# cv-stuttgart/PCFA

Measured on AMD Instinct MI355X. Metric: attack_steps_per_sec, higher is better.
Workload: dtype f32; 1 GPU; RAFT, 1 synthetic 436x1024 pair per GPU (padded 440x1024), disjoint delta, change_of_variables, delta_bound=0.005, zero target, L-BFGS max_iter=10; weights=random:1234, parallelism=pairs sharded 1/GPU, closure_launch=hipGraph replay

## Files before the change

include/pcfa_hip.h:

```cpp
#ifndef PCFA_HIP_H
#define PCFA_HIP_H

#include <stddef.h>
#include <stdint.h>

#ifdef __cplusplus
extern "C" {
#endif

#define PCFA_OK 0
#define PCFA_ERR_INVALID_ARG (-1)
#define PCFA_ERR_UNSUPPORTED (-2)
#define PCFA_ERR_WORKSPACE (-3)

#if defined(__GNUC__)
#define PCFA_API __attribute__((visibility("default")))
#else
#define PCFA_API
#endif

#define PCFA_MAX_LEVELS 8
#define PCFA_ABI_VERSION 2

#define PCFA_LOSS_AEE 0
// ... 82 lines not shown
                        int N, int d, float scale, void* stream);
PCFA_API int pcfa_attn_stream_delta(const float* g, const float* out, float* delta, long long rows, int d,
                           int accumulate, void* stream);
PCFA_API int pcfa_attn_stream_dqk(const float* q, const float* k, const float* lse, const float* G, const float* V,
                         const float* delta, float* dq, float* dk, int BH, int N, int d, int n, float scale,
                         void* stream);

PCFA_API long long pcfa_lookup_convc1_packed_floats(int Cout);
PCFA_API int pcfa_lookup_convc1_pack_weights(const float* weight, float* packed, int Cout, int Cin, void* stream);
PCFA_API int pcfa_lookup_convc1_fwd(const float* pyr, const float* coords, const float* packed, const float* bias,
                           float* out, int B, int H, int W, int num_levels, int radius, int Cout, int relu,
                           void* stream);
PCFA_API int pcfa_lookup_convc1_bwd(float* dpyr, const float* coords, const float* packed, const float* out,
                           const float* grad_out, int B, int H, int W, int num_levels, int radius, int Cout,
                           int relu, void* stream);

PCFA_API int pcfa_spatial_corr_out_size(int iH, int iW, int kH, int kW, int padH, int padW, int dilH,
                               int dilW, int dH, int dW, int* oH, int* oW);
PCFA_API int pcfa_spatial_corr_fwd(const float* in1, const float* in2, float* out, int B, int C, int iH,
                          int iW, int kH, int kW, int patchH, int patchW, int padH, int padW,
                          int dilH, int dilW, int dil_patchH, int dil_patchW, int dH, int dW,
                          void* stream);
PCFA_API int pcfa_spatial_corr_bwd(const float* in1, const float* in2, const float* grad_out,
                          float* grad_in1, float* grad_in2, int B, int C, int iH, int iW, int kH,
                          int kW, int patchH, int patchW, int padH, int padW, int dilH, int dilW,
                          int dil_patchH, int dil_patchW, int dH, int dW, void* stream);

PCFA_API int pcfa_cost_volume9_fwd(const float* in1, const float* in2, float* out, int B, int C, int iH, int iW,
                          float scale, float slope, void* stream);
PCFA_API int pcfa_cost_volume9_bwd(const float* in1, const float* in2, const float* fwd_out, const float* grad_out,
// ... 285 lines not shown
```

pcfa_amd/_hip.py:

```python
import ctypes
import os
from ctypes import c_char_p, c_double, c_float, c_int, c_longlong, c_size_t, c_uint, c_void_p, POINTER

ABI_VERSION = 2
LIB_PATH = os.environ.get("PCFA_HIP_LIB") or os.path.join(os.path.dirname(os.path.abspath(__file__)), "lib",
                                                          "libpcfa_hip.so")

PCFA_LOSS = {"aee": 0, "mse": 1, "cosim": 2}


class HipLibraryError(RuntimeError):
    pass


_P = c_void_p
_S4 = POINTER(c_longlong)

SIGNATURES = {
    "pcfa_abi_version": (c_int, []),
    "pcfa_timing_arm": (c_int, [_P, _P, c_int]),
    "pcfa_null_launch": (c_int, [_P]),
    "pcfa_poison_lds": (c_int, [c_uint, _P]),
    "pcfa_peek_lds": (c_int, [_P, c_int, _P]),
    "pcfa_calib_mfma_f32": (c_longlong, [_P, c_int, c_int, _P]),
# ... 27 lines not shown
    "pcfa_gemm_bf16x3_workspace_bytes": (c_size_t, [c_int, c_int, c_int, c_int]),
    "pcfa_gemm_bf16x3": (c_int, [_P, _P, _P, c_int, c_int, c_int, c_longlong, c_longlong, c_longlong, c_int, c_int,
                                 c_int, c_longlong, c_longlong, c_longlong, c_float, c_int, _P, c_size_t, _P]),
    "pcfa_corr_pyramid_fwd_bf16x3": (c_int, [_P, _P, _P, c_int, c_int, c_int, c_int, c_int, _P]),
    "pcfa_softmax_rows_fwd": (c_int, [_P, _P, c_longlong, c_int, _P]),
    "pcfa_softmax_rows_bwd": (c_int, [_P, _P, _P, c_longlong, c_int, _P]),
    "pcfa_attn_stream_lse": (c_int, [_P, _P, _P, c_int, c_int, c_int, c_float, _P]),
    "pcfa_attn_stream_fwd": (c_int, [_P, _P, _P, _P, _P, c_int, c_int, c_int, c_float, _P]),
    "pcfa_attn_stream_dv": (c_int, [_P, _P, _P, _P, _P, c_int, c_int, c_int, c_float, _P]),
    "pcfa_attn_stream_delta": (c_int, [_P, _P, _P, c_longlong, c_int, c_int, _P]),
    "pcfa_attn_stream_dqk": (c_int, [_P, _P, _P, _P, _P, _P, _P, _P, c_int, c_int, c_int, c_int, c_float, _P]),
    "pcfa_lookup_convc1_packed_floats": (c_longlong, [c_int]),
    "pcfa_lookup_convc1_pack_weights": (c_int, [_P, _P, c_int, c_int, _P]),
    "pcfa_lookup_convc1_fwd": (c_int, [_P, _P, _P, _P, _P, c_int, c_int, c_int, c_int, c_int, c_int, c_int, _P]),
    "pcfa_lookup_convc1_bwd": (c_int, [_P, _P, _P, _P, _P, c_int, c_int, c_int, c_int, c_int, c_int, c_int, _P]),
    "pcfa_spatial_corr_out_size": (c_int, [c_int] * 10 + [POINTER(c_int), POINTER(c_int)]),
    "pcfa_spatial_corr_fwd": (c_int, [_P, _P, _P] + [c_int] * 16 + [_P]),
    "pcfa_spatial_corr_bwd": (c_int, [_P, _P, _P, _P, _P] + [c_int] * 16 + [_P]),
    "pcfa_cost_volume9_fwd": (c_int, [_P, _P, _P, c_int, c_int, c_int, c_int, c_float, c_float, _P]),
    "pcfa_cost_volume9_bwd": (c_int, [_P, _P, _P, _P, _P, _P, c_int, c_int, c_int, c_int, c_float, c_float, _P]),
    "pcfa_flownet_corr_out_size": (c_int, [c_int] * 7 + [POINTER(c_int)] * 3),
    "pcfa_flownet_corr_fwd": (c_int, [_P, _P, _P] + [c_int] * 9 + [_P]),
    "pcfa_flownet_corr_bwd": (c_int, [_P, _P, _P, _P, _P] + [c_int] * 9 + [_P]),
    "pcfa_resample2d_fwd": (c_int, [_P, _P, _P] + [c_int] * 8 + [_P]),
    "pcfa_resample2d_bwd": (c_int, [_P, _P, _P, _P, _P] + [c_int] * 8 + [_P]),
    "pcfa_channelnorm_fwd": (c_int, [_P, _P, c_int, c_int, c_longlong, c_int, _P]),
    "pcfa_channelnorm_bwd": (c_int, [_P, _P, _P, _P, c_int, c_int, c_longlong, c_int, _P]),
    "pcfa_box_transform_fwd": (c_int, [_P, _P, _P, c_int, c_longlong, c_int, c_double, c_float, _P]),
    "pcfa_box_transform_bwd": (c_int, [_P, _P, _P, _P, _P, c_int, c_longlong, c_int, c_double, c_float, _P]),
    "pcfa_pm1_pair_fwd": (c_int, [_P, _P, _P, _P, c_int, c_longlong, _P]),
# ... 169 lines not shown
```

pcfa_amd/config.py:

```python
import dataclasses
import os


def _env_bool(name, default):
    v = os.environ.get(name)
    return default if v is None else v not in ("0", "", "false", "False")


@dataclasses.dataclass(frozen=True)
class Config:
    fused_lookup: bool = True
    overlap_encoders: bool = False
    conv_s2: bool = True
    conv_s2_bwd: bool = True
    fused_downsample: bool = True
    defer_relu: bool = True
    pyramid_bwd_windows: bool = True
    gma_gemm: str = "lib"
    gma_attention: str = "materialised"
    conv1x1: str = "lib"
    corr: str = "all_pairs"
    ondemand_lookup: str = "per_query"
    motion_bwd: str = "batched"
    mfma: str = "f32"
    dilated_as_subgrids: tuple = (2, 4, 8, 16)
    deconv_fewout: bool = True
    defer_leaky: bool = True
    dense_block_fused_masks: bool = True
    warp_bwd_deterministic: bool = True
    pwc_fold_glue: bool = True
    spynet_ops: str = "lib"
    flownet2_ops: str = "lib"
    reuse_pair_graphs: bool = True
    max_cached_shapes: int = 4

    @classmethod
    def from_env(cls):
        return cls(fused_lookup=_env_bool("PCFA_FUSED_LOOKUP", True),
# ... 11 lines not shown
                   max_cached_shapes=int(os.environ.get("PCFA_MAX_CACHED_SHAPES", "4")))

    def __post_init__(self):
        if self.gma_gemm not in ("lib", "hip"):
            raise ValueError("Config.gma_gemm must be 'lib' or 'hip', got %r" % (self.gma_gemm,))
        if self.gma_attention not in ("materialised", "streamed"):
            raise ValueError("Config.gma_attention must be 'materialised' or 'streamed', got %r" % (self.gma_attention,))
        if self.conv1x1 not in ("lib", "hip"):
            raise ValueError("Config.conv1x1 must be 'lib' or 'hip', got %r" % (self.conv1x1,))
        if self.corr not in ("all_pairs", "on_demand"):
            raise ValueError("Config.corr must be 'all_pairs' or 'on_demand', got %r" % (self.corr,))
        if self.ondemand_lookup not in ("per_query", "tiled"):
            raise ValueError("Config.ondemand_lookup must be 'per_query' or 'tiled', got %r" % (self.ondemand_lookup,))
        if self.motion_bwd not in ("batched", "per_iteration"):
            raise ValueError("Config.motion_bwd must be 'batched' or 'per_iteration', got %r" % (self.motion_bwd,))
        if self.mfma not in ("f32", "bf16x3"):
            raise ValueError("Config.mfma must be 'f32' or 'bf16x3', got %r" % (self.mfma,))
        if self.spynet_ops not in ("lib", "hip"):
            raise ValueError("Config.spynet_ops must be 'lib' or 'hip', got %r" % (self.spynet_ops,))
        if self.flownet2_ops not in ("lib", "hip"):
            raise ValueError("Config.flownet2_ops must be 'lib' or 'hip', got %r" % (self.flownet2_ops,))
        if self.max_cached_shapes < 1:
            raise ValueError("Config.max_cached_shapes must be >= 1")


DEFAULT = Config.from_env()


def attach(model, config=None):
    config = DEFAULT if config is None else config
# ... 10 lines not shown
```

pcfa_amd/csrc/corr_lookup_conv.hip:

```cpp
#include <cstdlib>
#include "common.hpp"

namespace {

typedef float f32x4 __attribute__((ext_vector_type(4)));
typedef float f32x16 __attribute__((ext_vector_type(16)));

constexpr int R = 4, N1 = 9, WIN = 10, TXN = 4, PIECES = WIN * TXN;
constexpr int RS = 20, WS = WIN * RS + 4, NRD = 3;
constexpr int QT = 32;
constexpr int NT = 256;
constexpr int NTF = NT + 64;
constexpr int NPC = QT * PIECES / NT;
constexpr int L = 4, TAPS = N1 * N1;
constexpr int KL = 88, KG = KL / 8;
constexpr int KP = L * KL;
constexpr int WIN_FLOATS = QT * WS + 4;
#ifndef PCFA_LC_WD
#define PCFA_LC_WD 8
#endif
#ifndef PCFA_LC_WDB
#define PCFA_LC_WDB 6
#endif
#ifndef PCFA_LC_EARLY
// ... 384 lines not shown
#pragma unroll
    for (int r = 0; r < 16; ++r) {
      const int n = (mt0 + m) * 32 + (r & 3) + 8 * (r >> 2) + 4 * lh;
      float y = acc[m][r];
      if (relu) y = fmaxf(y, 0.f);
      if (qlive) ob[(size_t)n * Q] = y;
    }
  if (dbg & 8) {
    PCFA_LC_STAMP();
    __syncthreads();
    if (tid == 0)
      for (int k = 0; k < 8; ++k) out[(size_t)b_img * COUT * Q + (size_t)k * Q + q0] = (float)(ts[k] - ts[0]);
  }
}

__global__ __launch_bounds__(NT) void corr_lookup_convc1_bwd_kernel(
    float* __restrict__ dpyr, const float* __restrict__ coords, const float* __restrict__ wt,
    const float* __restrict__ y, const float* __restrict__ grad_out, int Q, PyrLayout P, int relu) {
  constexpr int COUT = 256, MT = KP / 32;
  constexpr int MTW = 3;
  __shared__ __attribute__((aligned(16))) float s_a[COUT * QT > WIN_FLOATS ? COUT * QT : WIN_FLOATS];
  __shared__ __attribute__((aligned(16))) float s_dt[KP][QT];
  float (*s_g)[QT] = reinterpret_cast<float (*)[QT]>(s_a);
  float* s_win = s_a;

  const int tid = threadIdx.x, lane = tid & 63, wv = __builtin_amdgcn_readfirstlane(tid >> 6);
  const int j = tid & 31, l31 = lane & 31, lh = lane >> 5;
  const int b_img = blockIdx.z, q0 = blockIdx.x * QT;
  unsigned long long ts[12] = {};
  int nts = 0;
  constexpr int dbg = PCFA_LC_DBG_BUILD;
  PCFA_LC_STAMP();
  const int kq = tid >> 3, sub = tid & 7;
  const bool klive = q0 + kq < Q;
  const float* cb = coords + (size_t)b_img * 2 * Q;
  const int qj = min(q0 + j, Q - 1), qk = min(q0 + kq, Q - 1);
  const float cx = cb[qj], cy = cb[Q + qj], kx = cb[qk], ky = cb[Q + qk];
  float* slab0 = scalar_ptr(dpyr + ((size_t)b_img * Q + q0) * P.slab);

  const int qq = (tid & 7) * 4, n0 = tid >> 3;
  const size_t gbase = (size_t)b_img * COUT * Q + q0 + qq;
  const bool full = __builtin_amdgcn_readfirstlane((Q & 3) == 0 && q0 + QT <= Q);
  constexpr int NBLK = COUT / 32, AHEAD = PCFA_LC_AHEAD;
  f32x4 gg[NBLK], yy[NBLK];
  const float* ysrc = relu ? y : grad_out;
  const size_t glast = (size_t)gridDim.z * COUT * Q - 4;
  auto tile_load = [&](int i) {
    const size_t o = min(gbase + (size_t)(n0 + 32 * i) * Q, glast);
    gg[i] = *reinterpret_cast<const f32x4*>(grad_out + o);
    yy[i] = *reinterpret_cast<const f32x4*>(ysrc + o);
  };
  auto tile_store = [&](int i) {
    f32x4 t;
    t.x = (yy[i].x > 0.f || !relu) ? gg[i].x : 0.f; t.y = (yy[i].y > 0.f || !relu) ? gg[i].y : 0.f;
    t.z = (yy[i].z > 0.f || !relu) ? gg[i].z : 0.f; t.w = (yy[i].w > 0.f || !relu) ? gg[i].w : 0.f;
    *reinterpret_cast<f32x4*>(&s_g[n0 + 32 * i][qq]) = t;
  };
#pragma unroll
  for (int i = 0; i < AHEAD; ++i) tile_load(i);
  __builtin_amdgcn_sched_barrier(0);
// ... 25 lines not shown
    const int hl = Ph[l], wl = Pw[l], tw = Ptw[l], ox = org[l].ox;
    const int y = org[l].y0 + rr, gtx = (org[l].x0 >> 2) + tx;
    const bool need = (unsigned)y < (unsigned)hl && (unsigned)gtx < (unsigned)tw && 4 * tx < ox + WIN;
    const int c0 = 4 * tx - ox, gx0 = 4 * gtx;
    int mask = need ? 16 : 0;
#pragma unroll
    for (int e = 0; e < 4; ++e)
      if ((unsigned)(c0 + e) < (unsigned)WIN && gx0 + e < wl) mask |= 1 << e;
    pmask[l][i] = mask;
    pgoff[l][i] = need ? org[l].wB + (((((unsigned)y >> 2) * (unsigned)tw + (unsigned)gtx) << 4) + (((unsigned)y & 3u) << 2)) * 4u
                       : (unsigned)Pzero * 4u;
    plds[l][i] = (unsigned)(kq * WS + rr * RS + 4 + 4 * tx - ox) * 4u;
  };
  __builtin_amdgcn_sched_barrier(0);
  PCFA_LC_STAMP();
  if (!full) {
#pragma unroll 1
    for (int i = 0; i < NBLK; ++i) {
      const size_t o = gbase + (size_t)(n0 + 32 * i) * Q;
#pragma unroll
      for (int e = 0; e < 4; ++e) {
        const bool ok = q0 + qq + e < Q;
        const float gv = ok ? grad_out[o + e] : 0.f;
        const float yv = (ok && relu) ? y[o + e] : 1.f;
        s_g[n0 + 32 * i][qq + e] = yv > 0.f ? gv : 0.f;
      }
    }
  }

  {
    f32x16 acc[MTW];
#pragma unroll
    for (int m = 0; m < MTW; ++m)
#pragma unroll
      for (int r = 0; r < 16; ++r) acc[m][r] = 0.f;
    const f32x4* wq = reinterpret_cast<const f32x4*>(wt) + lane;
    const int nmt = wv + 8 < MT ? 3 : 2;
    constexpr int WD = PCFA_LC_WDB, NGB = COUT / 8;
    f32x4 wring[WD][MTW];
    size_t wrow[MTW];
#pragma unroll
    for (int m = 0; m < MTW; ++m) wrow[m] = (size_t)min(wv + 4 * m, MT - 1) * NGB;
#pragma unroll
    for (int d = 0; d < WD; ++d)
#pragma unroll
      for (int m = 0; m < MTW; ++m) wring[d][m] = wq[(wrow[m] + d) * 64];
    float bv[4] = {0.f, 0.f, 0.f, 0.f};
#pragma unroll
    for (int g = 0; g < NGB; ++g) {
      if (g % 4 == 0) {
        if (full) tile_store(g / 4);
        __syncthreads();
        if (g == 0) PCFA_LC_STAMP();
#pragma unroll
        for (int e = 0; e < 4; ++e) bv[e] = s_g[8 * g + 2 * e + lh][l31];
      }
      float bvn[4] = {0.f, 0.f, 0.f, 0.f};
      f32x4 wcur[MTW];
#pragma unroll
      for (int m = 0; m < MTW; ++m) wcur[m] = wring[g % WD][m];
#pragma unroll
      for (int e = 0; e < 4; ++e)
#pragma unroll
        for (int m = 0; m < MTW; ++m) {
          const int step = e * MTW + m;
          const float av = e == 0 ? wcur[m].x : e == 1 ? wcur[m].y : e == 2 ? wcur[m].z : wcur[m].w;
          acc[m] = __builtin_amdgcn_mfma_f32_32x32x2f32(av, bv[e], acc[m], 0, 0, 0);
          if (step == 0 && (g + 1) % 4 != 0) {
#pragma unroll
            for (int ee = 0; ee < 4; ++ee) bvn[ee] = s_g[8 * (g + 1) + 2 * ee + lh][l31];
          }
          if (step == 4 && g % 4 == 0 && g / 4 + AHEAD < NBLK) tile_load(g / 4 + AHEAD);
          if (step == 1 && g + WD < NGB) {
#pragma unroll
            for (int mm = 0; mm < MTW; ++mm) wring[g % WD][mm] = wq[(wrow[mm] + g + WD) * 64];
          }
          if (step == 2 && g < L * NPC && g % NPC == 0) level_setup(g / NPC);
          if (step == 3 && g < L * NPC) piece_setup(g / NPC, g % NPC);
          if (step == 5 && g < L * NPC) v[g / NPC][g % NPC] = load_piece(slab0, pgoff[g / NPC][g % NPC]);
          __builtin_amdgcn_sched_barrier(0);
        }
#pragma unroll
      for (int e = 0; e < 4; ++e) bv[e] = bvn[e];
    }
#pragma unroll
    for (int m = 0; m < MTW; ++m) {
      if (m < nmt) {
#pragma unroll
        for (int r = 0; r < 16; ++r)
          s_dt[(wv + 4 * m) * 32 + (r & 3) + 8 * (r >> 2) + 4 * lh][l31] = acc[m][r];
      }
    }
  }
  __syncthreads();
  PCFA_LC_STAMP();

#pragma unroll
  for (int l = 0; l < L; ++l) {
    const Origin oj = make_origin(cx, cy, l);
    const float fx = oj.fx, fy = oj.fy;
    const float w00 = (1.f - fx) * (1.f - fy), w01 = fx * (1.f - fy), w10 = (1.f - fx) * fy, w11 = fx * fy;
#pragma unroll
    for (int pass = 0; pass < 2; ++pass) {
      const int row = pass == 0 ? (tid >> 5) : 8;
      if (pass == 1 && tid >= 32) break;
      float gc[N1], gp[N1];
#pragma unroll
      for (int a = 0; a < N1; ++a) {
        gc[a] = s_dt[l * KL + a * N1 + row][j];
        gp[a] = row > 0 ? s_dt[l * KL + a * N1 + row - 1][j] : 0.f;
      }
      float4* dst0 = reinterpret_cast<float4*>(&s_win[j * WS + row * RS + 4]);
      float d[NRD * 4];
#pragma unroll
      for (int c = 0; c < NRD * 4; ++c) {
        float s = 0.f;
        if (c < N1) s = gc[c] * w00;
        if (c >= 1 && c <= N1) s = fmaf(gc[c - 1], w01, s);
        if (c < N1) s = fmaf(gp[c], w10, s);
        if (c >= 1 && c <= N1) s = fmaf(gp[c - 1], w11, s);
        d[c] = s;
      }
#pragma unroll
      for (int i = 0; i < NRD; ++i) dst0[i] = make_float4(d[4 * i], d[4 * i + 1], d[4 * i + 2], d[4 * i + 3]);
      if (row == N1 - 1) {
        float4* dst1 = reinterpret_cast<float4*>(&s_win[j * WS + (WIN - 1) * RS + 4]);
#pragma unroll
        for (int c = 0; c < NRD * 4; ++c) {
          float s = 0.f;
          if (c < N1) s = gc[c] * w10;
          if (c >= 1 && c <= N1) s = fmaf(gc[c - 1], w11, s);
          d[c] = s;
        }
#pragma unroll
        for (int i = 0; i < NRD; ++i) dst1[i] = make_float4(d[4 * i], d[4 * i + 1], d[4 * i + 2], d[4 * i + 3]);
      }
    }
    __syncthreads();
    const char* lds_bytes = reinterpret_cast<const char*>(s_win);
#pragma unroll
    for (int i = 0; i < NPC; ++i) {
      const float* src = reinterpret_cast<const float*>(lds_bytes + plds[l][i]);
      const float e0 = src[0], e1 = src[1], e2 = src[2], e3 = src[3];
      const int m = pmask[l][i];
      f32x4 t = v[l][i];
      t.x += (m & 1) ? e0 : 0.f;
      t.y += (m & 2) ? e1 : 0.f;
      t.z += (m & 4) ? e2 : 0.f;
      t.w += (m & 8) ? e3 : 0.f;
      if (m & 16) store_piece(slab0, pgoff[l][i], t);
    }
    __syncthreads();
    PCFA_LC_STAMP();
  }
  if (dbg & 8) {
    if (tid == 0)
      for (int k = 0; k < 8; ++k) slab0[k] = (float)(ts[k] - ts[0]);
  }
}

bool check_levels(const PyrLayout& P) {
  for (int l = 0; l < P.L; ++l)
    if (P.h[l] < 1 || P.w[l] < 1 || P.h[l] > 32000 || P.w[l] > 32000) return false;
  return true;
}

}

extern "C" long long pcfa_lookup_convc1_packed_floats(int Cout) {
  if (Cout != 256) return -1;
  return 2LL * Cout * KP;
}

// ... 23 lines not shown

extern "C" int pcfa_lookup_convc1_bwd(float* dpyr, const float* coords, const float* packed, const float* out,
                                      const float* grad_out, int B, int H, int W, int num_levels, int radius,
                                      int Cout, int relu, void* stream) {
  PyrLayout P;
  if (!dpyr || !coords || !packed || !out || !grad_out || B < 1 || !pcfa_make_layout(P, H, W, num_levels) ||
      !check_levels(P))
    return PCFA_ERR_INVALID_ARG;
  if (num_levels != L || radius != R || Cout != 256) return PCFA_ERR_UNSUPPORTED;
  const int Q = H * W;
  pcfa_launch(corr_lookup_convc1_bwd_kernel, dim3(pcfa_cdiv(Q, QT), 1, B), dim3(NT), 0, (hipStream_t)stream, dpyr,
              coords, packed + (size_t)Cout * KP, out, grad_out, Q, P, relu);
  PCFA_LAUNCH_CHECK();
  return PCFA_OK;
}
```

pcfa_amd/nets/raft.py:

```python

import torch
import torch.nn as nn
import torch.nn.functional as F

from .. import ops
from ..config import cfg


def _norm(kind, planes):
    if kind == 'batch':
        return nn.BatchNorm2d(planes)
    if kind == 'instance':
        return nn.InstanceNorm2d(planes)
    if kind == 'group':
        return nn.GroupNorm(num_groups=planes // 8, num_channels=planes)
    if kind == 'none':
        return nn.Sequential()
    raise ValueError("unknown norm_fn %r" % kind)


def _fold_batchnorm(conv, bn, cache, tag):
    tensors = (conv.weight, conv.bias, bn.weight, bn.bias, bn.running_mean, bn.running_var)
    key = tuple((t.data_ptr(), t._version) for t in tensors if t is not None) + (conv.weight.device,)
    hit = cache.get(tag)
# ... 359 lines not shown
class BasicUpdateBlock(nn.Module):
    def __init__(self, corr_levels=4, corr_radius=4, hidden_dim=128):
        super().__init__()
        self.encoder = BasicMotionEncoder(corr_levels, corr_radius)
        self.gru = SepConvGRU(hidden_dim=hidden_dim, input_dim=128 + hidden_dim)
        self.flow_head = FlowHead(hidden_dim, hidden_dim=256)
        self.mask = _mask_head()
        self._mask_cache = {}

    def motion_steps(self, corr_fn, flow, iters, gru_ctx):
        c, enc = cfg(self), self.encoder
        make = getattr(ops.get(), "motion_steps", None)
        if (make is None or c.motion_bwd != "batched" or not c.defer_relu or not c.fused_lookup or c.corr == "on_demand"
                or gru_ctx is None or not flow.is_cuda or not enc.can_defer_relu(flow)):
            return None
        return make(corr_fn, iters, *((m.weight, m.bias) for m in (enc.convc1, enc.convc2, enc.convf1, enc.convf2, enc.conv)))

    def forward(self, net, inp, corr, flow, want_mask=True, gru_ctx=None, motion=None):
        if motion is not None:
            steps, itr = motion
            net = self.gru.step(net, gru_ctx, steps.step(itr, corr.coords, flow), self.encoder.RELU_CHANNELS,
                                d_rest_dst=steps.d_rest_dst(itr))
        else:
            defer = cfg(self).defer_relu and gru_ctx is not None and self.encoder.can_defer_relu(flow)
            motion_features = self.encoder(flow, corr, defer_relu=defer)
            if gru_ctx is not None:
                net = self.gru.step(net, gru_ctx, motion_features, self.encoder.RELU_CHANNELS if defer else 0)
            else:
                net = self.gru(net, torch.cat([inp, motion_features], dim=1))
        delta_flow = self.flow_head(net)
        mask = mask_logits(self.mask, net, self._mask_cache) if want_mask else None
# ... 91 lines not shown
```

pcfa_amd/ops/corr.py:

```python
import ctypes
import os

import torch

from .. import _hip
from . import core
from .conv import FEWIN_SHAPES, _conv3x3_cat_fill, _conv3x3_packed, _conv3x3_run, conv_fewin
from .core import _call, _dev, _note_work, _pair, _ptr, _ptr_off, _stream, cached_pack


class _CorrState:
    __slots__ = ("B", "D", "H", "W", "L", "r", "slab", "pyr", "f2ext", "dpyr", "token_grad", "coords_bwd", "bwd_windows", "mfma")


class _CorrBuild(torch.autograd.Function):

    @staticmethod
    def forward(ctx, fmap1, fmap2, state):
        lib = _hip.load()
        B, D, H, W = fmap1.shape
        f1 = fmap1.contiguous()
        f2 = fmap2.contiguous()
        slab = state.slab
        state.f2ext = torch.empty((B, D, slab), device=f1.device, dtype=torch.float32)
# ... 122 lines not shown
        if ctx.needs_input_grad[3] or ctx.needs_input_grad[4]:
            raise RuntimeError("lookup_conv is the frozen-weight path: no weight / bias gradient")
        st = ctx.state
        c, out = ctx.saved_tensors
        if st.dpyr is None:
            st.dpyr = torch.zeros_like(st.pyr)
            st.coords_bwd = []
        st.coords_bwd.append(c)
        g = grad_out.contiguous()
        _call("pcfa_lookup_convc1_bwd", _ptr(st.dpyr), _ptr(c), _ptr(ctx.packed), _ptr(out), _ptr(g), st.B, st.H, st.W,
              st.L, st.r, ctx.cout, ctx.relu)
        return _token_grad(st, g.device), None, None, None, None, None


class _MotionState:
    __slots__ = ("iters", "H", "W", "corr", "w", "cor1", "cf", "rest", "d_rest", "coords", "arrived", "token_grad", "packs")


def _slab_image(slab, i):
    n = slab[0].numel()
    return torch.empty(0, device=slab.device, dtype=slab.dtype).set_(
        slab.untyped_storage(), slab.storage_offset() + i * n, (1,) + tuple(slab.shape[1:]))


class _MotionFlush(torch.autograd.Function):

    @staticmethod
    def forward(ctx, token, ms):
        ctx.ms = ms
        return token.view_as(token)

# ... 15 lines not shown
        direct = lambda b, k, n_: (lib.pcfa_conv3x3_algo(b, k, n_, H, W) == 23
                                   and lib.pcfa_conv3x3_workspace_bytes(b, k, n_, H, W) == 0)
        batched = (len(live) == n and all(direct(b, k, n_) for b in (1, n)
                                          for k, n_ in ((n_c, k_c), (n_c, n_c2), (n_c2, k_c2))))
        d_cor1 = torch.empty((n, k_c2, H, W), device=dev, dtype=torch.float32)
        if batched:
            d_cf = torch.empty((n, n_c2, H, W), device=dev, dtype=torch.float32)
            _call("pcfa_conv3x3_run_strided", _ptr(ms.d_rest), wr * plane, _ptr(bwd_c), None, _ptr(ms.cf), k_c * plane, None, 0,
                  _ptr(d_cf), n_c2 * plane, n, n_c, n_c2, H, W, 0, 0., 0, None, ctypes.c_size_t(0))
            _call("pcfa_conv3x3_run_strided", _ptr(d_cf), n_c2 * plane, _ptr(bwd_c2), None, _ptr(ms.cor1), k_c2 * plane, None, 0,
                  _ptr(d_cor1), k_c2 * plane, n, n_c2, k_c2, H, W, 0, 0., 0, None, ctypes.c_size_t(0))
        if st.dpyr is None:
            st.dpyr = torch.zeros_like(st.pyr)
            st.coords_bwd = []
        packed = _convc1_packed(ms.w["convc1"][0])
        for i in reversed(live):
            if not batched:
                d_cf = torch.empty((1, k_c, H, W), device=dev, dtype=torch.float32)
                _conv3x3_run(dev, _ptr_off(ms.d_rest, i * wr * plane), bwd_c, None, _ptr_off(ms.cf, i * k_c * plane), None,
                             _ptr(d_cf), 1, n_c, k_c, H, W)
                _conv3x3_run(dev, _ptr(d_cf), bwd_c2, None, _ptr_off(ms.cor1, i * k_c2 * plane), None,
                             _ptr_off(d_cor1, i * k_c2 * plane), 1, n_c2, k_c2, H, W)
            st.coords_bwd.append(ms.coords[i])
            _call("pcfa_lookup_convc1_bwd", _ptr(st.dpyr), _ptr(ms.coords[i]), _ptr(packed), _ptr_off(ms.cor1, i * k_c2 * plane),
                  _ptr_off(d_cor1, i * k_c2 * plane), st.B, st.H, st.W, st.L, st.r, k_c2, 1)
        return grad_token, None


class _MotionStep(torch.autograd.Function):

    @staticmethod
    def forward(ctx, token, coords, flow, ms, i):
        st = ms.corr
        c = coords.contiguous()
        (wc1, bc1), (wc2, bc2), (wf1, bf1), (wf2, bf2), (wc, bc) = (ms.w[k] for k in ("convc1", "convc2", "convf1", "convf2", "conv"))
        cor1, cf, rest = _slab_image(ms.cor1, i), _slab_image(ms.cf, i), _slab_image(ms.rest, i)
        _call("pcfa_lookup_convc1_fwd", _ptr(st.pyr), _ptr(c), _ptr(_convc1_packed(wc1)), _ptr(bc1), _ptr(cor1), st.B, st.H,
              st.W, st.L, st.r, wc1.shape[0], 1)
        flo1 = conv_fewin(flow, wf1, bf1, True)
        _conv3x3_cat_fill([cor1, flo1.contiguous()], [wc2, wf2], [bc2, bf2], (), cf)
# ... 24 lines not shown
        self._ms, self._token = ms, token

    def step(self, i, coords, flow):
        _dev(coords, flow)
        if coords.requires_grad and torch.is_grad_enabled():
            raise RuntimeError("motion_steps: coords.requires_grad is not supported (detach the coordinates, as "
                               "models/raft/raft.py:122-123 does)")
        if flow.requires_grad and torch.is_grad_enabled():
            raise RuntimeError("motion_steps: the flow must be detached (models/raft/raft.py:122-123)")
        return _MotionStep.apply(self._token, coords, flow, self._ms, i)

    def d_rest_dst(self, i):
        return _slab_image(self._ms.d_rest, i)


def motion_steps(corr_block, iters, convc1, convc2, convf1, convf2, conv):
    if not isinstance(corr_block, CorrBlock) or iters < 1:
        return None
    st = corr_block._state
    (wc1, bc1), (wc2, bc2), (wf1, bf1), (wf2, bf2), (wc, bc) = convc1, convc2, convf1, convf2, conv
    if (st.B != 1 or st.L != 4 or st.r != 4 or bc1 is None or tuple(wc1.shape) != (256, 324, 1, 1)
            or not corr_block._token.requires_grad
            or any(t is None or t.requires_grad for t in (wc1, bc1, wc2, bc2, wf1, bf1, wf2, bf2, wc, bc))
            or any(tuple(w.shape[2:]) != (3, 3) for w in (wc2, wf2, wc))
            or (wf1.shape[1], wf1.shape[2]) not in FEWIN_SHAPES or wf1.shape[2] != wf1.shape[3]
            or wc2.shape[1] != wc1.shape[0] or wf2.shape[1] != wf1.shape[0] or wc.shape[1] != wc2.shape[0] + wf2.shape[0]):
        return None
    dev = st.pyr.device
    ms = _MotionState()
    ms.iters, ms.H, ms.W, ms.corr = iters, st.H, st.W, st
    ms.w = {"convc1": convc1, "convc2": convc2, "convf1": convf1, "convf2": convf2, "conv": conv}
    new = lambda c: torch.empty((iters, c, st.H, st.W), device=dev, dtype=torch.float32)
    ms.cor1, ms.cf = new(wc1.shape[0]), new(wc.shape[1])
    ms.rest, ms.d_rest = new(wc.shape[0] + 2), new(wc.shape[0] + 2)
    ms.coords, ms.arrived, ms.token_grad = [None] * iters, [False] * iters, None
    ms.packs = ((_conv3x3_packed(wc)[1], wc.shape[1], wc.shape[0]), (_conv3x3_packed(wc2)[1], wc2.shape[1], wc2.shape[0]))
    return MotionSteps(ms, _MotionFlush.apply(corr_block._token, ms))


class CorrBlock:

    def __init__(self, fmap1, fmap2, num_levels=4, radius=4, bwd_windows=True, mfma="f32"):
        _dev(fmap1, fmap2)
        if mfma not in ("f32", "bf16x3"):
            raise ValueError("CorrBlock: mfma must be 'f32' or 'bf16x3', got %r" % (mfma,))
        if fmap1.shape != fmap2.shape or fmap1.dim() != 4:
            raise ValueError("CorrBlock expects two [B,D,H,W] feature maps of equal shape")
        lib = _hip.load()
        self.num_levels = num_levels
        self.radius = radius
# ... 136 lines not shown
```

Before: 7.891 attack_steps/s.

## Fuse per-iteration lookup-convc1 backward launches into one multi-step kernel

Adds a multi-step variant of the lookup+convc1 backward kernel that loops over all RAFT iterations inside one launch. Each block keeps its dpyr slab tile resident and prefetches the next step's coords, gradient tiles and weight ring while it finishes the current step's scatter. This replaces roughly one launch per GRU iteration with a single launch and overlaps the step prologues. In exchange the kernel carries a larger by-value argument struct, extra fences, and more register pressure. It only applies when B==1 and there are at most 32 steps.

```diff
diff --git a/include/pcfa_hip.h b/include/pcfa_hip.h
--- a/include/pcfa_hip.h
+++ b/include/pcfa_hip.h
@@ -120,6 +120,9 @@
 PCFA_API int pcfa_lookup_convc1_bwd(float* dpyr, const float* coords, const float* packed, const float* out,
                            const float* grad_out, int B, int H, int W, int num_levels, int radius, int Cout,
                            int relu, void* stream);
+PCFA_API int pcfa_lookup_convc1_bwd_steps(float* dpyr, const float* const* coords, const long long* offsets,
+                           int nsteps, const float* packed, const float* out, const float* grad_out, int B, int H,
+                           int W, int num_levels, int radius, int Cout, int relu, void* stream);
 
 PCFA_API int pcfa_spatial_corr_out_size(int iH, int iW, int kH, int kW, int padH, int padW, int dilH,
                                int dilW, int dH, int dW, int* oH, int* oW);
diff --git a/pcfa_amd/_hip.py b/pcfa_amd/_hip.py
--- a/pcfa_amd/_hip.py
+++ b/pcfa_amd/_hip.py
@@ -65,6 +65,8 @@
     "pcfa_lookup_convc1_pack_weights": (c_int, [_P, _P, c_int, c_int, _P]),
     "pcfa_lookup_convc1_fwd": (c_int, [_P, _P, _P, _P, _P, c_int, c_int, c_int, c_int, c_int, c_int, c_int, _P]),
     "pcfa_lookup_convc1_bwd": (c_int, [_P, _P, _P, _P, _P, c_int, c_int, c_int, c_int, c_int, c_int, c_int, _P]),
+    "pcfa_lookup_convc1_bwd_steps": (c_int, [_P, POINTER(c_void_p), POINTER(c_longlong), c_int, _P, _P, _P, c_int, c_int,
+                                             c_int, c_int, c_int, c_int, c_int, _P]),
     "pcfa_spatial_corr_out_size": (c_int, [c_int] * 10 + [POINTER(c_int), POINTER(c_int)]),
     "pcfa_spatial_corr_fwd": (c_int, [_P, _P, _P] + [c_int] * 16 + [_P]),
     "pcfa_spatial_corr_bwd": (c_int, [_P, _P, _P, _P, _P] + [c_int] * 16 + [_P]),
diff --git a/pcfa_amd/config.py b/pcfa_amd/config.py
--- a/pcfa_amd/config.py
+++ b/pcfa_amd/config.py
@@ -22,6 +22,7 @@
     corr: str = "all_pairs"
     ondemand_lookup: str = "per_query"
     motion_bwd: str = "batched"
+    lookup_bwd: str = "steps"
     mfma: str = "f32"
     dilated_as_subgrids: tuple = (2, 4, 8, 16)
     deconv_fewout: bool = True
@@ -63,6 +64,8 @@
             raise ValueError("Config.ondemand_lookup must be 'per_query' or 'tiled', got %r" % (self.ondemand_lookup,))
         if self.motion_bwd not in ("batched", "per_iteration"):
             raise ValueError("Config.motion_bwd must be 'batched' or 'per_iteration', got %r" % (self.motion_bwd,))
+        if self.lookup_bwd not in ("steps", "per_iteration"):
+            raise ValueError("Config.lookup_bwd must be 'steps' or 'per_iteration', got %r" % (self.lookup_bwd,))
         if self.mfma not in ("f32", "bf16x3"):
             raise ValueError("Config.mfma must be 'f32' or 'bf16x3', got %r" % (self.mfma,))
         if self.spynet_ops not in ("lib", "hip"):
diff --git a/pcfa_amd/csrc/corr_lookup_conv.hip b/pcfa_amd/csrc/corr_lookup_conv.hip
--- a/pcfa_amd/csrc/corr_lookup_conv.hip
+++ b/pcfa_amd/csrc/corr_lookup_conv.hip
@@ -422,9 +422,29 @@
   }
 }
 
-__global__ __launch_bounds__(NT) void corr_lookup_convc1_bwd_kernel(
-    float* __restrict__ dpyr, const float* __restrict__ coords, const float* __restrict__ wt,
-    const float* __restrict__ y, const float* __restrict__ grad_out, int Q, PyrLayout P, int relu) {
+constexpr int MAX_STEPS = 32;
+struct OneStep {
+  const float *coords_, *y_, *grad_;
+  __device__ __forceinline__ int count() const { return 1; }
+  __device__ __forceinline__ const float* coords(int) const { return coords_; }
+  __device__ __forceinline__ const float* y(int) const { return y_; }
+  __device__ __forceinline__ const float* grad(int) const { return grad_; }
+};
+struct LookupSteps {
+  const float* coords_[MAX_STEPS];
+  long long off[MAX_STEPS];
+  const float *y_, *grad_;
+  int n;
+  __device__ __forceinline__ int count() const { return n; }
+  __device__ __forceinline__ const float* coords(int s) const { return coords_[s]; }
+  __device__ __forceinline__ const float* y(int s) const { return y_ + off[s]; }
+  __device__ __forceinline__ const float* grad(int s) const { return grad_ + off[s]; }
+};
+
+template <bool STEPS, typename Src>
+__device__ __forceinline__ void lookup_convc1_bwd_body(float* __restrict__ dpyr, const Src& src,
+                                                       const float* __restrict__ wt, int Q, const PyrLayout& P,
+                                                       int relu) {
   constexpr int COUT = 256, MT = KP / 32;
   constexpr int MTW = 3;
   __shared__ __attribute__((aligned(16))) float s_a[COUT * QT > WIN_FLOATS ? COUT * QT : WIN_FLOATS];
@@ -437,13 +457,21 @@
   const int b_img = blockIdx.z, q0 = blockIdx.x * QT;
   unsigned long long ts[12] = {};
   int nts = 0;
-  constexpr int dbg = PCFA_LC_DBG_BUILD;
+  constexpr int dbg = STEPS ? (PCFA_LC_DBG_BUILD & ~8) : PCFA_LC_DBG_BUILD;
   PCFA_LC_STAMP();
   const int kq = tid >> 3, sub = tid & 7;
   const bool klive = q0 + kq < Q;
-  const float* cb = coords + (size_t)b_img * 2 * Q;
   const int qj = min(q0 + j, Q - 1), qk = min(q0 + kq, Q - 1);
-  const float cx = cb[qj], cy = cb[Q + qj], kx = cb[qk], ky = cb[Q + qk];
+  const int nsteps = STEPS ? __builtin_amdgcn_readfirstlane(src.count()) : 1;
+  float cx, cy, kx, ky;
+  float ncx = 0.f, ncy = 0.f, nkx = 0.f, nky = 0.f;
+  auto coords_load = [&](int s, float& ax, float& ay, float& bx, float& by) {
+    const float* cb = src.coords(s) + (size_t)b_img * 2 * Q;
+    ax = cb[qj]; ay = cb[Q + qj]; bx = cb[qk]; by = cb[Q + qk];
+  };
+  coords_load(0, cx, cy, kx, ky);
+  const float* grad_out = src.grad(0);
+  const float* y = src.y(0);
   float* slab0 = scalar_ptr(dpyr + ((size_t)b_img * Q + q0) * P.slab);
 
   const int qq = (tid & 7) * 4, n0 = tid >> 3;
@@ -452,6 +480,11 @@
   constexpr int NBLK = COUT / 32, AHEAD = PCFA_LC_AHEAD;
   f32x4 gg[NBLK], yy[NBLK];
   const float* ysrc = relu ? y : grad_out;
+  auto step_sources = [&](int s) {
+    grad_out = src.grad(s);
+    y = src.y(s);
+    ysrc = relu ? y : grad_out;
+  };
   const size_t glast = (size_t)gridDim.z * COUT * Q - 4;
   auto tile_load = [&](int i) {
     const size_t o = min(gbase + (size_t)(n0 + 32 * i) * Q, glast);
@@ -507,149 +540,191 @@
   };
   __builtin_amdgcn_sched_barrier(0);
   PCFA_LC_STAMP();
-  if (!full) {
+  constexpr int WD = PCFA_LC_WDB, NGB = COUT / 8;
+  const f32x4* wq = reinterpret_cast<const f32x4*>(wt) + lane;
+  const int nmt = wv + 8 < MT ? 3 : 2;
+  f32x4 wring[WD][MTW];
+  size_t wrow[MTW];
+#pragma unroll
+  for (int m = 0; m < MTW; ++m) wrow[m] = (size_t)min(wv + 4 * m, MT - 1) * NGB;
+  auto ring_fill = [&]() {
+    if (STEPS) asm volatile("" : "+v"(wq));
+#pragma unroll
+    for (int d = 0; d < WD; ++d)
+#pragma unroll
+      for (int m = 0; m < MTW; ++m) wring[d][m] = wq[(wrow[m] + d) * 64];
+  };
+
 #pragma unroll 1
-    for (int i = 0; i < NBLK; ++i) {
-      const size_t o = gbase + (size_t)(n0 + 32 * i) * Q;
-#pragma unroll
-      for (int e = 0; e < 4; ++e) {
-        const bool ok = q0 + qq + e < Q;
-        const float gv = ok ? grad_out[o + e] : 0.f;
-        const float yv = (ok && relu) ? y[o + e] : 1.f;
-        s_g[n0 + 32 * i][qq + e] = yv > 0.f ? gv : 0.f;
+  for (int s = 0; s < nsteps; ++s) {
+    if (!full) {
+#pragma unroll 1
+      for (int i = 0; i < NBLK; ++i) {
+        const size_t o = gbase + (size_t)(n0 + 32 * i) * Q;
+#pragma unroll
+        for (int e = 0; e < 4; ++e) {
+          const bool ok = q0 + qq + e < Q;
+          const float gv = ok ? grad_out[o + e] : 0.f;
+          const float yv = (ok && relu) ? y[o + e] : 1.f;
+          s_g[n0 + 32 * i][qq + e] = yv > 0.f ? gv : 0.f;
+        }
       }
     }
-  }
-
-  {
-    f32x16 acc[MTW];
-#pragma unroll
-    for (int m = 0; m < MTW; ++m)
-#pragma unroll
-      for (int r = 0; r < 16; ++r) acc[m][r] = 0.f;
-    const f32x4* wq = reinterpret_cast<const f32x4*>(wt) + lane;
-    const int nmt = wv + 8 < MT ? 3 : 2;
-    constexpr int WD = PCFA_LC_WDB, NGB = COUT / 8;
-    f32x4 wring[WD][MTW];
-    size_t wrow[MTW];
-#pragma unroll
-    for (int m = 0; m < MTW; ++m) wrow[m] = (size_t)min(wv + 4 * m, MT - 1) * NGB;
-#pragma unroll
-    for (int d = 0; d < WD; ++d)
-#pragma unroll
-      for (int m = 0; m < MTW; ++m) wring[d][m] = wq[(wrow[m] + d) * 64];
-    float bv[4] = {0.f, 0.f, 0.f, 0.f};
-#pragma unroll
-    for (int g = 0; g < NGB; ++g) {
-      if (g % 4 == 0) {
-        if (full) tile_store(g / 4);
-        __syncthreads();
-        if (g == 0) PCFA_LC_STAMP();
-#pragma unroll
-        for (int e = 0; e < 4; ++e) bv[e] = s_g[8 * g + 2 * e + lh][l31];
+
+    {
+      f32x16 acc[MTW];
+#pragma unroll
+      for (int m = 0; m < MTW; ++m)
+#pragma unroll
+        for (int r = 0; r < 16; ++r) acc[m][r] = 0.f;
+      if (!STEPS || s == 0) ring_fill();
+      float bv[4] = {0.f, 0.f, 0.f, 0.f};
+#pragma unroll
+      for (int g = 0; g < NGB; ++g) {
+        if (g % 4 == 0) {
+          if (full) tile_store(g / 4);
+          __syncthreads();
+          if (g == 0) PCFA_LC_STAMP();
+#pragma unroll
+          for (int e = 0; e < 4; ++e) bv[e] = s_g[8 * g + 2 * e + lh][l31];
+        }
+        float bvn[4] = {0.f, 0.f, 0.f, 0.f};
+        f32x4 wcur[MTW];
+#pragma unroll
+        for (int m = 0; m < MTW; ++m) wcur[m] = wring[g % WD][m];
+#pragma unroll
+        for (int e = 0; e < 4; ++e)
+#pragma unroll
+          for (int m = 0; m < MTW; ++m) {
+            const int step = e * MTW + m;
+            const float av = e == 0 ? wcur[m].x : e == 1 ? wcur[m].y : e == 2 ? wcur[m].z : wcur[m].w;
+            acc[m] = __builtin_amdgcn_mfma_f32_32x32x2f32(av, bv[e], acc[m], 0, 0, 0);
+            if (step == 0 && (g + 1) % 4 != 0) {
+#pragma unroll
+              for (int ee = 0; ee < 4; ++ee) bvn[ee] = s_g[8 * (g + 1) + 2 * ee + lh][l31];
+            }
+            if (step == 4 && g % 4 == 0 && g / 4 + AHEAD < NBLK) tile_load(g / 4 + AHEAD);
+            if (step == 1 && g + WD < NGB) {
+#pragma unroll
+              for (int mm = 0; mm < MTW; ++mm) wring[g % WD][mm] = wq[(wrow[mm] + g + WD) * 64];
+            }
+            if (step == 2 && g < L * NPC && g % NPC == 0) level_setup(g / NPC);
+            if (step == 3 && g < L * NPC) piece_setup(g / NPC, g % NPC);
+            if (step == 5 && g < L * NPC) v[g / NPC][g % NPC] = load_piece(slab0, pgoff[g / NPC][g % NPC]);
+            __builtin_amdgcn_sched_barrier(0);
+          }
+#pragma unroll
+        for (int e = 0; e < 4; ++e) bv[e] = bvn[e];
       }
-      float bvn[4] = {0.f, 0.f, 0.f, 0.f};
-      f32x4 wcur[MTW];
-#pragma unroll
-      for (int m = 0; m < MTW; ++m) wcur[m] = wring[g % WD][m];
-#pragma unroll
-      for (int e = 0; e < 4; ++e)
-#pragma unroll
-        for (int m = 0; m < MTW; ++m) {
-          const int step = e * MTW + m;
-          const float av = e == 0 ? wcur[m].x : e == 1 ? wcur[m].y : e == 2 ? wcur[m].z : wcur[m].w;
-          acc[m] = __builtin_amdgcn_mfma_f32_32x32x2f32(av, bv[e], acc[m], 0, 0, 0);
-          if (step == 0 && (g + 1) % 4 != 0) {
-#pragma unroll
-            for (int ee = 0; ee < 4; ++ee) bvn[ee] = s_g[8 * (g + 1) + 2 * ee + lh][l31];
-          }
-          if (step == 4 && g % 4 == 0 && g / 4 + AHEAD < NBLK) tile_load(g / 4 + AHEAD);
-          if (step == 1 && g + WD < NGB) {
-#pragma unroll
-            for (int mm = 0; mm < MTW; ++mm) wring[g % WD][mm] = wq[(wrow[mm] + g + WD) * 64];
-          }
-          if (step == 2 && g < L * NPC && g % NPC == 0) level_setup(g / NPC);
-          if (step == 3 && g < L * NPC) piece_setup(g / NPC, g % NPC);
-          if (step == 5 && g < L * NPC) v[g / NPC][g % NPC] = load_piece(slab0, pgoff[g / NPC][g % NPC]);
-          __builtin_amdgcn_sched_barrier(0);
+#pragma unroll
+      for (int m = 0; m < MTW; ++m) {
+        if (m < nmt) {
+#pragma unroll
+          for (int r = 0; r < 16; ++r)
+            s_dt[(wv + 4 * m) * 32 + (r & 3) + 8 * (r >> 2) + 4 * lh][l31] = acc[m][r];
         }
-#pragma unroll
-      for (int e = 0; e < 4; ++e) bv[e] = bvn[e];
-    }
-#pragma unroll
-    for (int m = 0; m < MTW; ++m) {
-      if (m < nmt) {
-#pragma unroll
-        for (int r = 0; r < 16; ++r)
-          s_dt[(wv + 4 * m) * 32 + (r & 3) + 8 * (r >> 2) + 4 * lh][l31] = acc[m][r];
       }
     }
-  }
-  __syncthreads();
-  PCFA_LC_STAMP();
-
-#pragma unroll
-  for (int l = 0; l < L; ++l) {
-    const Origin oj = make_origin(cx, cy, l);
-    const float fx = oj.fx, fy = oj.fy;
-    const float w00 = (1.f - fx) * (1.f - fy), w01 = fx * (1.f - fy), w10 = (1.f - fx) * fy, w11 = fx * fy;
-#pragma unroll
-    for (int pass = 0; pass < 2; ++pass) {
-      const int row = pass == 0 ? (tid >> 5) : 8;
-      if (pass == 1 && tid >= 32) break;
-      float gc[N1], gp[N1];
-#pragma unroll
-      for (int a = 0; a < N1; ++a) {
-        gc[a] = s_dt[l * KL + a * N1 + row][j];
-        gp[a] = row > 0 ? s_dt[l * KL + a * N1 + row - 1][j] : 0.f;
-      }
-      float4* dst0 = reinterpret_cast<float4*>(&s_win[j * WS + row * RS + 4]);
-      float d[NRD * 4];
-#pragma unroll
-      for (int c = 0; c < NRD * 4; ++c) {
-        float s = 0.f;
-        if (c < N1) s = gc[c] * w00;
-        if (c >= 1 && c <= N1) s = fmaf(gc[c - 1], w01, s);
-        if (c < N1) s = fmaf(gp[c], w10, s);
-        if (c >= 1 && c <= N1) s = fmaf(gp[c - 1], w11, s);
-        d[c] = s;
-      }
-#pragma unroll
-      for (int i = 0; i < NRD; ++i) dst0[i] = make_float4(d[4 * i], d[4 * i + 1], d[4 * i + 2], d[4 * i + 3]);
-      if (row == N1 - 1) {
-        float4* dst1 = reinterpret_cast<float4*>(&s_win[j * WS + (WIN - 1) * RS + 4]);
+    __syncthreads();
+    PCFA_LC_STAMP();
+
+    const bool more = STEPS && s + 1 < nsteps;
+    if (more) {
+      step_sources(s + 1);
+      coords_load(s + 1, ncx, ncy, nkx, nky);
+#pragma unroll
+      for (int i = 0; i < AHEAD; ++i) tile_load(i);
+      ring_fill();
+      __builtin_amdgcn_sched_barrier(0);
+    }
+
+    if (dbg & 32) {
+      if (s_dt[tid][0] == 12345.678f && v[0][0].x == 8765.4321f) slab0[0] = 1.f;
+      __syncthreads();
+    }
+#pragma unroll
+    for (int l = 0; l < ((dbg & 32) ? 0 : L); ++l) {
+      const Origin oj = make_origin(cx, cy, l);
+      const float fx = oj.fx, fy = oj.fy;
+      const float w00 = (1.f - fx) * (1.f - fy), w01 = fx * (1.f - fy), w10 = (1.f - fx) * fy, w11 = fx * fy;
+#pragma unroll
+      for (int pass = 0; pass < 2; ++pass) {
+        const int row = pass == 0 ? (tid >> 5) : 8;
+        if (pass == 1 && tid >= 32) break;
+        float gc[N1], gp[N1];
+#pragma unroll
+        for (int a = 0; a < N1; ++a) {
+          gc[a] = s_dt[l * KL + a * N1 + row][j];
+          gp[a] = row > 0 ? s_dt[l * KL + a * N1 + row - 1][j] : 0.f;
+        }
+        float4* dst0 = reinterpret_cast<float4*>(&s_win[j * WS + row * RS + 4]);
+        float d[NRD * 4];
 #pragma unroll
         for (int c = 0; c < NRD * 4; ++c) {
           float s = 0.f;
-          if (c < N1) s = gc[c] * w10;
-          if (c >= 1 && c <= N1) s = fmaf(gc[c - 1], w11, s);
+          if (c < N1) s = gc[c] * w00;
+          if (c >= 1 && c <= N1) s = fmaf(gc[c - 1], w01, s);
+          if (c < N1) s = fmaf(gp[c], w10, s);
+          if (c >= 1 && c <= N1) s = fmaf(gp[c - 1], w11, s);
           d[c] = s;
         }
 #pragma unroll
-        for (int i = 0; i < NRD; ++i) dst1[i] = make_float4(d[4 * i], d[4 * i + 1], d[4 * i + 2], d[4 * i + 3]);
+        for (int i = 0; i < NRD; ++i) dst0[i] = make_float4(d[4 * i], d[4 * i + 1], d[4 * i + 2], d[4 * i + 3]);
+        if (row == N1 - 1) {
+          float4* dst1 = reinterpret_cast<float4*>(&s_win[j * WS + (WIN - 1) * RS + 4]);
+#pragma unroll
+          for (int c = 0; c < NRD * 4; ++c) {
+            float s = 0.f;
+            if (c < N1) s = gc[c] * w10;
+            if (c >= 1 && c <= N1) s = fmaf(gc[c - 1], w11, s);
+            d[c] = s;
+          }
+#pragma unroll
+          for (int i = 0; i < NRD; ++i) dst1[i] = make_float4(d[4 * i], d[4 * i + 1], d[4 * i + 2], d[4 * i + 3]);
+        }
       }
-    }
-    __syncthreads();
-    const char* lds_bytes = reinterpret_cast<const char*>(s_win);
-#pragma unroll
-    for (int i = 0; i < NPC; ++i) {
-      const float* src = reinterpret_cast<const float*>(lds_bytes + plds[l][i]);
-      const float e0 = src[0], e1 = src[1], e2 = src[2], e3 = src[3];
-      const int m = pmask[l][i];
-      f32x4 t = v[l][i];
-      t.x += (m & 1) ? e0 : 0.f;
-      t.y += (m & 2) ? e1 : 0.f;
-      t.z += (m & 4) ? e2 : 0.f;
-      t.w += (m & 8) ? e3 : 0.f;
-      if (m & 16) store_piece(slab0, pgoff[l][i], t);
-    }
-    __syncthreads();
-    PCFA_LC_STAMP();
+      __syncthreads();
+      const char* lds_bytes = reinterpret_cast<const char*>(s_win);
+#pragma unroll
+      for (int i = 0; i < NPC; ++i) {
+        const float* src = reinterpret_cast<const float*>(lds_bytes + plds[l][i]);
+        const float e0 = src[0], e1 = src[1], e2 = src[2], e3 = src[3];
+        const int m = pmask[l][i];
+        f32x4 t = v[l][i];
+        t.x += (m & 1) ? e0 : 0.f;
+        t.y += (m & 2) ? e1 : 0.f;
+        t.z += (m & 4) ? e2 : 0.f;
+        t.w += (m & 8) ? e3 : 0.f;
+        if (m & 16) store_piece(slab0, pgoff[l][i], t);
+      }
+      if (more && l == L - 1) {
+        asm volatile("s_waitcnt vmcnt(0)" ::: "memory");
+        __builtin_amdgcn_fence(__ATOMIC_RELEASE, "workgroup");
+      }
+      __syncthreads();
+      if (more && l == L - 1) __builtin_amdgcn_fence(__ATOMIC_ACQUIRE, "workgroup");
+      PCFA_LC_STAMP();
+    }
+    if (more) {
+      cx = ncx; cy = ncy; kx = nkx; ky = nky;
+    }
   }
   if (dbg & 8) {
     if (tid == 0)
       for (int k = 0; k < 8; ++k) slab0[k] = (float)(ts[k] - ts[0]);
   }
+}
+
+__global__ __launch_bounds__(NT) void corr_lookup_convc1_bwd_kernel(
+    float* __restrict__ dpyr, const float* __restrict__ coords, const float* __restrict__ wt,
+    const float* __restrict__ y, const float* __restrict__ grad_out, int Q, PyrLayout P, int relu) {
+  const OneStep one = {coords, y, grad_out};
+  lookup_convc1_bwd_body<false>(dpyr, one, wt, Q, P, relu);
+}
+
+__global__ __launch_bounds__(NT) void corr_lookup_convc1_steps_bwd_kernel(
+    float* __restrict__ dpyr, LookupSteps steps, const float* __restrict__ wt, int Q, PyrLayout P, int relu) {
+  lookup_convc1_bwd_body<true>(dpyr, steps, wt, Q, P, relu);
 }
 
 bool check_levels(const PyrLayout& P) {
@@ -703,3 +778,28 @@
   PCFA_LAUNCH_CHECK();
   return PCFA_OK;
 }
+
+extern "C" int pcfa_lookup_convc1_bwd_steps(float* dpyr, const float* const* coords, const long long* offsets,
+                                            int nsteps, const float* packed, const float* out, const float* grad_out,
+                                            int B, int H, int W, int num_levels, int radius, int Cout, int relu,
+                                            void* stream) {
+  PyrLayout P;
+  if (!dpyr || !coords || !offsets || !packed || !out || !grad_out || B < 1 || nsteps < 1 ||
+      !pcfa_make_layout(P, H, W, num_levels) || !check_levels(P))
+    return PCFA_ERR_INVALID_ARG;
+  if (num_levels != L || radius != R || Cout != 256 || nsteps > MAX_STEPS) return PCFA_ERR_UNSUPPORTED;
+  LookupSteps steps = {};
+  for (int s = 0; s < nsteps; ++s) {
+    if (!coords[s] || offsets[s] < 0) return PCFA_ERR_INVALID_ARG;
+    steps.coords_[s] = coords[s];
+    steps.off[s] = offsets[s];
+  }
+  steps.y_ = out;
+  steps.grad_ = grad_out;
+  steps.n = nsteps;
+  const int Q = H * W;
+  pcfa_launch(corr_lookup_convc1_steps_bwd_kernel, dim3(pcfa_cdiv(Q, QT), 1, B), dim3(NT), 0, (hipStream_t)stream,
+              dpyr, steps, packed + (size_t)Cout * KP, Q, P, relu);
+  PCFA_LAUNCH_CHECK();
+  return PCFA_OK;
+}
diff --git a/pcfa_amd/nets/raft.py b/pcfa_amd/nets/raft.py
--- a/pcfa_amd/nets/raft.py
+++ b/pcfa_amd/nets/raft.py
@@ -397,7 +397,8 @@
         if (make is None or c.motion_bwd != "batched" or not c.defer_relu or not c.fused_lookup or c.corr == "on_demand"
                 or gru_ctx is None or not flow.is_cuda or not enc.can_defer_relu(flow)):
             return None
-        return make(corr_fn, iters, *((m.weight, m.bias) for m in (enc.convc1, enc.convc2, enc.convf1, enc.convf2, enc.conv)))
+        return make(corr_fn, iters, *((m.weight, m.bias) for m in (enc.convc1, enc.convc2, enc.convf1, enc.convf2, enc.conv)),
+                    lookup_bwd=c.lookup_bwd)
 
     def forward(self, net, inp, corr, flow, want_mask=True, gru_ctx=None, motion=None):
         if motion is not None:
diff --git a/pcfa_amd/ops/corr.py b/pcfa_amd/ops/corr.py
--- a/pcfa_amd/ops/corr.py
+++ b/pcfa_amd/ops/corr.py
@@ -160,7 +160,8 @@
 
 
 class _MotionState:
-    __slots__ = ("iters", "H", "W", "corr", "w", "cor1", "cf", "rest", "d_rest", "coords", "arrived", "token_grad", "packs")
+    __slots__ = ("iters", "H", "W", "corr", "w", "cor1", "cf", "rest", "d_rest", "coords", "arrived", "token_grad", "packs",
+                 "lookup_bwd")
 
 
 def _slab_image(slab, i):
@@ -206,7 +207,9 @@
             st.dpyr = torch.zeros_like(st.pyr)
             st.coords_bwd = []
         packed = _convc1_packed(ms.w["convc1"][0])
-        for i in reversed(live):
+        order = list(reversed(live))
+        steps = ms.lookup_bwd == "steps" and len(order) <= 32 and st.B == 1
+        for i in order:
             if not batched:
                 d_cf = torch.empty((1, k_c, H, W), device=dev, dtype=torch.float32)
                 _conv3x3_run(dev, _ptr_off(ms.d_rest, i * wr * plane), bwd_c, None, _ptr_off(ms.cf, i * k_c * plane), None,
@@ -214,8 +217,15 @@
                 _conv3x3_run(dev, _ptr(d_cf), bwd_c2, None, _ptr_off(ms.cor1, i * k_c2 * plane), None,
                              _ptr_off(d_cor1, i * k_c2 * plane), 1, n_c2, k_c2, H, W)
             st.coords_bwd.append(ms.coords[i])
-            _call("pcfa_lookup_convc1_bwd", _ptr(st.dpyr), _ptr(ms.coords[i]), _ptr(packed), _ptr_off(ms.cor1, i * k_c2 * plane),
-                  _ptr_off(d_cor1, i * k_c2 * plane), st.B, st.H, st.W, st.L, st.r, k_c2, 1)
+            if not steps:
+                _call("pcfa_lookup_convc1_bwd", _ptr(st.dpyr), _ptr(ms.coords[i]), _ptr(packed),
+                      _ptr_off(ms.cor1, i * k_c2 * plane), _ptr_off(d_cor1, i * k_c2 * plane), st.B, st.H, st.W, st.L, st.r,
+                      k_c2, 1)
+        if steps:
+            ptrs = (ctypes.c_void_p * len(order))(*[ms.coords[i].data_ptr() for i in order])
+            offs = (ctypes.c_longlong * len(order))(*[i * k_c2 * plane for i in order])
+            _call("pcfa_lookup_convc1_bwd_steps", _ptr(st.dpyr), ptrs, offs, len(order), _ptr(packed), _ptr(ms.cor1),
+                  _ptr(d_cor1), st.B, st.H, st.W, st.L, st.r, k_c2, 1)
         return grad_token, None
 
 
@@ -270,7 +280,7 @@
         return _slab_image(self._ms.d_rest, i)
 
 
-def motion_steps(corr_block, iters, convc1, convc2, convf1, convf2, conv):
+def motion_steps(corr_block, iters, convc1, convc2, convf1, convf2, conv, lookup_bwd="steps"):
     if not isinstance(corr_block, CorrBlock) or iters < 1:
         return None
     st = corr_block._state
@@ -290,6 +300,7 @@
     ms.cor1, ms.cf = new(wc1.shape[0]), new(wc.shape[1])
     ms.rest, ms.d_rest = new(wc.shape[0] + 2), new(wc.shape[0] + 2)
     ms.coords, ms.arrived, ms.token_grad = [None] * iters, [False] * iters, None
+    ms.lookup_bwd = lookup_bwd
     ms.packs = ((_conv3x3_packed(wc)[1], wc.shape[1], wc.shape[0]), (_conv3x3_packed(wc2)[1], wc2.shape[1], wc2.shape[0]))
     return MotionSteps(ms, _MotionFlush.apply(corr_block._token, ms))
 
```

Measured after the change: 7.907 attack_steps/s, median of 6. No clear change (+0.2%).
